# gergely-flamich/compression-without-quantization

Measured on AMD Instinct MI355X. Metric: latent blocks encoded/s at KL=16 bits, higher is better.
Workload: dtype f32

## Files before the change

### compression_without_quantization_amd/build.py

```python
import os
import subprocess
import sys

HERE = os.path.dirname(os.path.abspath(__file__))
CSRC = os.path.join(HERE, "csrc")
OUT = os.path.join(HERE, "libcwq.so")
SOURCES = ["cwq_kernels.hip", "cwq_importance.hip", "cwq_pln.hip", "cwq_partition.hip",
           "cwq_varbits.hip", "cwq_capi.hip", "cwq_ac.cpp"]
HEADERS = ["cwq_math.h", "cwq_screen.h", "cwq_dispatch.h", "cwq_kernels.h", "cwq_device.h",
           "cwq_debug.h"]

FLAGS = ["--offload-arch=gfx950", "-O3", "-std=c++17", "-ffp-contract=off", "-fno-fast-math",
         "-fPIC", "-shared", "-Wall", "-Wno-unused-function"]
LIBS = ["-L/opt/rocm/lib", "-lhsa-runtime64"]


def _stale():
    if not os.path.exists(OUT):
        return True
    t = os.path.getmtime(OUT)
    deps = [os.path.join(CSRC, f) for f in SOURCES + HEADERS]
    deps.append(os.path.join(HERE, "..", "include", "cwq.h"))
    deps.append(os.path.abspath(__file__))
    return any(os.path.getmtime(p) > t for p in deps if os.path.exists(p))


def build(force=False, verbose=True):
    if not force and not _stale():
        return OUT
    cmd = ["hipcc"] + FLAGS + ["-o", OUT] + [os.path.join(CSRC, s) for s in SOURCES] + LIBS
    if verbose:
        print(" ".join(cmd), flush=True)
    subprocess.check_call(cmd)
    return OUT


if __name__ == "__main__":
    build(force="--force" in sys.argv)
```

### compression_without_quantization_amd/csrc/cwq_kernels.hip

```cpp
#include <hip/hip_runtime.h>

#include <type_traits>
#include <stdint.h>

#include "cwq_device.h"
#include "cwq_kernels.h"

namespace cwq {

__global__ void __launch_bounds__(256) k_prep_dims(
    const float* __restrict__ t_scale, const float* __restrict__ p_loc,
    const float* __restrict__ p_scale, int64_t n, float nst, float sdiv, float rho,
    float* __restrict__ loc_s, float* __restrict__ scale_s, float* __restrict__ lognorm,
    float* __restrict__ out_sample, unsigned long long* __restrict__ keys, int64_t nb) {
  for (int64_t g = blockIdx.x * (int64_t)blockDim.x + threadIdx.x; g < nb;
       g += (int64_t)gridDim.x * blockDim.x)
    keys[g] = 0ull;
  for (int64_t i = blockIdx.x * (int64_t)blockDim.x + threadIdx.x; i < n;
       i += (int64_t)gridDim.x * blockDim.x) {
    float ls, ss;
    shard_consts(p_loc[i], p_scale[i], nst, sdiv, rho, ls, ss);
    loc_s[i] = ls;
    scale_s[i] = ss;
    lognorm[i] = lognorm_of(t_scale[i]);
    out_sample[i] = 0.0f;
  }
}

template <int DC, bool STEP0>
__device__ __forceinline__ float eval_row(const PhiloxStream& st, uint64_t kbase, int64_t d_rt,
                                          int align_rt, const float* __restrict__ loc_s,
                                          const float* __restrict__ scale_s,
                                          const float* __restrict__ mu,
                                          const float* __restrict__ sg,
                                          const float* __restrict__ lognorm,
                                          const float* __restrict__ best,
                                          const double* logtab) {
  return eval_row_f<DC>(st, kbase, d_rt, align_rt, logtab, [&](int64_t e, float zz) -> float {
    float s = scale_s[e] * zz;
    s = loc_s[e] + s;
    const float tv = STEP0 ? s : best[e] + s;
    return log_prob(tv, mu[e], sg[e], lognorm[e]);
  });
}

template <int DC, bool STEP0>
__global__ void __launch_bounds__(256) k_encode_eval(
    const float* __restrict__ t_loc, const float* __restrict__ t_scale,
    const float* __restrict__ loc_s, const float* __restrict__ scale_s,
    const float* __restrict__ lognorm, const float* __restrict__ best,
    const int64_t* __restrict__ block_off, int64_t ud, int64_t ntiles, int64_t tiles_per_block,
    int64_t cand_per_tile, int64_t n_cand, SeedSpec sd, int32_t step,
    unsigned long long* __restrict__ keys) {
  __shared__ double logtab[32];
  __shared__ unsigned long long wkey[4];
  fill_logtab(logtab);
  const uint32_t wv = wave_id();
  const uint32_t lane = threadIdx.x & 63u;

  for (int64_t tile = blockIdx.x; tile < ntiles; tile += gridDim.x) {
    const int64_t g = tile / tiles_per_block;
    const int64_t tt = tile - g * tiles_per_block;
    const BlockSpan sp = block_span(block_off, ud, g);
    const int64_t n0 = tt * cand_per_tile;
    const int64_t n1 = (n0 + cand_per_tile < n_cand) ? n0 + cand_per_tile : n_cand;
    const PhiloxStream st =
        generate_key(step_seed(sd.of(g), step), 42);
    const int align = (int)(((uint64_t)(n0 + wv) * (uint64_t)sp.d) & 3u);

    uint64_t bestk = 0;
    for (int64_t n = n0 + 4 * (int64_t)lane + wv; n < n1; n += 256) {
      const float v = eval_row<DC, STEP0>(st, (uint64_t)n * (uint64_t)sp.d, sp.d, align,
                                          loc_s + sp.off, scale_s + sp.off, t_loc + sp.off,
                                          t_scale + sp.off, lognorm + sp.off,
                                          STEP0 ? nullptr : best + sp.off, logtab);
      const uint64_t k = argmax_key(v, (uint32_t)n);
      bestk = k > bestk ? k : bestk;
    }
    bestk = wave_max_u64(bestk);
    if (lane == 0) wkey[wv] = bestk;
    __syncthreads();
    if (threadIdx.x == 0) {
      uint64_t m = wkey[0];
      for (int i = 1; i < 4; ++i) m = wkey[i] > m ? wkey[i] : m;
      if (m) atomicMax(&keys[g], (unsigned long long)m);
    }
    __syncthreads();
  }
}

constexpr float kPruneC1 = 0x1p-14f;
#ifndef CWQ_PRUNE_MIN_WAVES
#define CWQ_PRUNE_MIN_WAVES 6
#endif
#ifndef CWQ_XCD_BALANCE
#define CWQ_XCD_BALANCE 1
#endif
#ifndef CWQ_TAU_SHARE_MASK
#define CWQ_TAU_SHARE_MASK 7u
#endif
#ifndef CWQ_CSR_TAU_SHARE_MASK
#define CWQ_CSR_TAU_SHARE_MASK 15u
#endif
#ifndef CWQ_SURVIVOR_CAP
#define CWQ_SURVIVOR_CAP 1024
#endif

template <bool STEP0>
__device__ __forceinline__ float cand_diff(float z, float ls, float ss, float mu, float bb) {
  const float s = shard_sample(ls, ss, z);
  const float tv = STEP0 ? s : bb + s;
  return tv - mu;
}
__device__ __forceinline__ float lp_from_z(float z, float cc) {
  const float u = -0.5f * (z * z);
  return u - cc;
}


struct VisitRec {
  float4 sa, sb;
  int grp;
  int bk;
  int pad[2];
};
static_assert(sizeof(VisitRec) == 48, "VisitRec: 48 bytes");

template <int D, bool STEP0>
__device__ __forceinline__ float score_rows_wave(
    const PhiloxStream& st, const uint32_t* rows, uint32_t cnt, const float* __restrict__ loc_s,
    const float* __restrict__ scale_s, const float* __restrict__ mu,
    const float* __restrict__ sg, const float* __restrict__ lognorm,
    const float* __restrict__ best, const double* logtab, float* buf, uint32_t lane) {
  constexpr uint32_t G = D / 4;
  const uint32_t r = lane / G, u = lane - r * G;
  if (r < cnt) {
    const F4 z = normal4_dev(st, (uint64_t)rows[r] * G + u, logtab);
#pragma unroll
    for (int t = 0; t < 4; ++t) {
      const uint32_t j = 4u * u + (uint32_t)t;
      const float zz = t == 0 ? z.a : (t == 1 ? z.b : (t == 2 ? z.c : z.d));
      float v = scale_s[j] * zz;
      v = loc_s[j] + v;
      const float tv = STEP0 ? v : best[j] + v;
      buf[r * D + j] = log_prob(tv, mu[j], sg[j], lognorm[j]);
    }
  }
  __builtin_amdgcn_fence(__ATOMIC_SEQ_CST, "wavefront");
  __builtin_amdgcn_wave_barrier();
  float acc = 0.0f;
  const uint32_t fr = lane >> 3;
  if (fr < cnt)
    for (uint32_t e = lane & 7u; e < (uint32_t)D; e += 8u) acc = acc + buf[fr * D + e];
  __builtin_amdgcn_fence(__ATOMIC_SEQ_CST, "wavefront");
  __builtin_amdgcn_wave_barrier();
  float p[8];
#pragma unroll
  for (int l = 0; l < 8; ++l) p[l] = __shfl(acc, (int)((lane & ~7u) + (uint32_t)l), 64);
  return eigen_fold8(p, 0.0f);
}

#ifdef CWQ_TILE_TIMES
constexpr int kTileTimes = 1 << 18;
__device__ unsigned long long g_tile_t0[kTileTimes], g_tile_t1[kTileTimes];
__device__ unsigned int g_tile_wg[kTileTimes];
#endif
#ifdef CWQ_PRUNE_STATS
__device__ unsigned long long g_prune_stats[72];
constexpr int kDbgBlocks = 1 << 20;
__device__ unsigned long long g_dbg_best[kDbgBlocks];
__device__ int g_seed_tau;
#endif

template <int D, bool STEP0, bool INTER>
__global__ void __launch_bounds__(256, CWQ_PRUNE_MIN_WAVES) k_encode_prune(
    const float* __restrict__ t_loc, const float* __restrict__ t_scale,
    const float* __restrict__ loc_s, const float* __restrict__ scale_s,
    const float* __restrict__ lognorm, const float* __restrict__ best, int64_t ntiles,
    int64_t tiles_per_block, int64_t cand_per_tile, int64_t n_cand, SeedSpec sd, int32_t step,
    int allow_screen, unsigned long long* __restrict__ keys, int64_t tail_from, int tail_div,
    uint32_t* __restrict__ tq) {
  static_assert(D % 8 == 0 && D >= 8 && D <= 64, "pruned path: D % 8 == 0, D <= 64");
  constexpr int G = D / 4;
  constexpr int NF = STEP0 ? 6 : 7;
  constexpr int RW = (64 / G) < 8 ? (64 / G) : 8;
  __shared__ double logtab[32];
  __shared__ float4 cst[G * NF];
  __shared__ VisitRec vrec[G];
  __shared__ int2 meta[G];
  __shared__ float rowbuf[4][RW * D];
  __shared__ float dscore[D];
  __shared__ float dA[D];
  __shared__ float dC[D];
  __shared__ float gscore[G];
  __shared__ int gpos[G];
  __shared__ float lowc;
  __shared__ float scr_a, scr_pq;
  __shared__ float tau_cell;
  __shared__ uint32_t sq_cnt;
  __shared__ uint32_t sq_n[CWQ_SURVIVOR_CAP];
  __shared__ float sq_ub[CWQ_SURVIVOR_CAP];
  __shared__ unsigned long long wkey[4];
  __shared__ uint32_t s_next;
#ifdef CWQ_PRUNE_STATS
  __shared__ uint32_t s_ps[72];
  for (int i = threadIdx.x; i < 72; i += blockDim.x) s_ps[i] = 0u;
#endif
  fill_logtab(logtab);
  const uint32_t wv = wave_id();
  const uint32_t lane = threadIdx.x & 63u;

  constexpr bool inter = INTER;
  const int64_t nbt = INTER ? ntiles / tiles_per_block : 0;
  auto next_tile = [&](int64_t cur) -> int64_t {
    if (tq == nullptr) return cur + gridDim.x;
    __syncthreads();
    if (threadIdx.x == 0) s_next = gridDim.x + atomicAdd(tq, 1u);
    __syncthreads();
    return (int64_t)s_next;
  };
  for (int64_t tile = blockIdx.x; tile < ntiles; tile = next_tile(tile)) {
    uint32_t tid = threadIdx.x;
    asm volatile("" : "+v"(tid));
#ifdef CWQ_TILE_TIMES
    if (tid == 0 && tile < kTileTimes) {
      g_tile_t0[tile] = __builtin_amdgcn_s_memrealtime();
      const uint32_t xcc = (uint32_t)__builtin_amdgcn_s_getreg((20) | (0 << 6) | ((4 - 1) << 11));
      g_tile_wg[tile] = (xcc << 24) | (blockIdx.x & 0xffffffu);
    }
#endif
    int64_t tord = tile;
    const int64_t treg = inter ? nbt * tail_from : 0;
    if (inter && CWQ_XCD_BALANCE && tq == nullptr && tile < treg && (treg & 7) == 0 &&
        (gridDim.x & 7u) == 0)
      tord = (tile & 7) * (treg >> 3) + (tile >> 3);
    const int64_t g = inter ? tord % nbt : tile / tiles_per_block;
    const int64_t tt = inter ? tord / nbt : tile - g * tiles_per_block;
    const int64_t off = g * D;
    int64_t n0, csz;
    if (tt < tail_from) {
      n0 = tt * cand_per_tile;
      csz = cand_per_tile;
    } else {
      csz = cand_per_tile / tail_div;
      n0 = tail_from * cand_per_tile + (tt - tail_from) * csz;
    }
    const int64_t n1 = (n0 + csz < n_cand) ? n0 + csz : n_cand;
    if (n0 >= n1) continue;
    const PhiloxStream st =
        generate_key(step_seed(sd.of(g), step), 42);

    if (tid < D) {
      const int j = tid;
      const float ls = loc_s[off + j], ss = scale_s[off + j], mu = t_loc[off + j];
      const float rs = 1.0f / t_scale[off + j];
      const float m = (STEP0 ? ls : best[off + j] + ls) - mu;
      float e = 0.5f * (ss * ss + m * m) * (rs * rs);
      dscore[j] = (e == e) ? e : -1.0f;
    }
    __syncthreads();
    if (tid < G) {
      const int q = tid;
      gscore[q] = ((dscore[4 * q] + dscore[4 * q + 1]) + dscore[4 * q + 2]) + dscore[4 * q + 3];
    }
    __syncthreads();
    if (tid < G) {
      const int q = tid;
      const float sq = gscore[q];
      int r = 0;
      for (int q2 = 0; q2 < G; ++q2) {
        const float s2 = gscore[q2];
        r += (s2 > sq || (s2 == sq && q2 < q)) ? 1 : 0;
      }
      gpos[q] = r;
      meta[r].x = q;
      vrec[r].grp = q;
    }
    __syncthreads();
    int den_ok = 1, scr_ok = 1;
    if (tid < D) {
      const int j = tid, k = gpos[j >> 2], w = j & 3;
      float fj[7];
      const float sgj = t_scale[off + j];
      fj[0] = loc_s[off + j];
      fj[1] = scale_s[off + j];
      fj[2] = t_loc[off + j];
      fj[3] = sgj;
      fj[4] = lognorm[off + j];
      fj[5] = 1.0f / sgj;
      fj[6] = STEP0 ? 0.0f : best[off + j];
      float* c = reinterpret_cast<float*>(cst);
#pragma unroll
      for (int f = 0; f < NF; ++f) c[(k * NF + f) * 4 + w] = fj[f];
      den_ok = markstein_ok_den(sgj) ? 1 : 0;
      const ScreenDim o = screen_dim<STEP0>(fj[0], fj[1], fj[2], sgj, fj[4], fj[6]);
      float* sc = reinterpret_cast<float*>(&vrec[k]);
      sc[w] = o.sa;
      sc[4 + w] = o.sb;
      dA[j] = o.A;
      dC[j] = o.C;
      scr_ok = o.ok ? 1 : 0;
    }
    const bool fastdiv = __syncthreads_and(den_ok) != 0;
    const bool scr_all = __syncthreads_and(scr_ok) != 0;
    const bool screen = allow_screen && scr_all;
    if (tid <= G + 1) {
      const int kb = tid;
      const float* c = reinterpret_cast<const float*>(cst);
      double rf = 0.0, kk = 0.0, asum = 0.0, msum = 0.0, kall = 0.0, cvis = 0.0, a2 = 0.0,
             amax = 0.0;
#pragma unroll 1
      for (int p = 0; p < D; ++p) {
        const double mj = -(double)c[((p >> 2) * NF + 4) * 4 + (p & 3)];
        const double aj = __builtin_fabs(mj);
        asum += aj;
        msum += mj;
        kall += aj + mj;
        if (p >= 4 * kb) {
          rf += mj + 0x1p-17 * aj;
        } else {
          kk += aj + mj;
          if (screen) cvis += (double)dC[(meta[p >> 2].x << 2) + (p & 3)];
        }
        if (screen && kb == G + 1) {
          const double av = (double)dA[p];
          a2 += av * av;
          amax = av > amax ? av : amax;
        }
      }
      const double marg = 0x1p-20 * (__builtin_fabs(rf) + asum) + 0x1p-126;
      const double sl = 0x1p-14 * (__builtin_fabs(msum) + asum + kall) + 0x1p-126;
      if (kb <= G) {
        const float bk = screen ? round_up_f32(msum + cvis * (1.0 + 0x1p-20) + sl)
                                : round_up_f32(rf + 0x1p-14 * kk + marg);
        if (kb >= 1) {
          meta[kb - 1].y = (int)f2u(bk);
          vrec[kb - 1].bk = (int)f2u(bk);
        }
        if (kb == G) lowc = round_up_f32(0x1p-14 * kk + marg);
      } else if (screen) {
        scr_a = screen_as(msum, sl, a2);
        scr_pq = screen_pq(amax, D);
      }
      if (kb == 0) {
        float t0 = -__builtin_inff();
        if (inter) {
          const unsigned long long kv =
              __hip_atomic_load(&keys[g], __ATOMIC_RELAXED, __HIP_MEMORY_SCOPE_AGENT);
          if ((uint32_t)(kv >> 32) > kArgmaxClampOrd) t0 = unord_f32((uint32_t)(kv >> 32));
        }
#ifdef CWQ_PRUNE_STATS
        if (g_seed_tau && g < kDbgBlocks && (g_dbg_best[g] >> 32) > kArgmaxClampOrd)
          t0 = unord_f32((uint32_t)(g_dbg_best[g] >> 32));
#endif
        tau_cell = t0;
        sq_cnt = 0u;
      }
    }
    __syncthreads();
    const float lc = lowc;
#ifdef CWQ_PRUNE_STATS
    const float tau_seed = tau_cell;
#endif
    const float sA = scr_a, sPq = scr_pq;

    const int64_t per_wave = (n1 - n0 + 3) / 4;
    const int64_t w0 = n0 + (int64_t)wv * per_wave;
    const int64_t w1 = (w0 + per_wave < n1) ? w0 + per_wave : n1;
    const uint32_t w0g =
        (uint32_t)__builtin_amdgcn_readfirstlane((int)((uint32_t)w0 * (uint32_t)G));
    const uint32_t ng_end = (uint32_t)__builtin_amdgcn_readfirstlane(
        (int)(w1 > w0 ? (uint32_t)(w1 - w0) * (uint32_t)G : 0u));
#ifndef CWQ_TAU_FROM_KEYS
#define CWQ_TAU_FROM_KEYS 1
#endif
    float tau = (INTER && CWQ_TAU_FROM_KEYS) ? tau_cell : -__builtin_inff();
#ifdef CWQ_PRUNE_STATS
    tau = tau_seed;
#endif
    uint64_t bestk = 0;

    const PhiloxLo lok = philox_lo_key(st);
    auto pass = [&](auto screen_tag) {
      constexpr bool SCREEN = decltype(screen_tag)::value;
      constexpr uint32_t KS = SCREEN ? (uint32_t)sizeof(VisitRec) : 1u;
      uint32_t ng = lane * (uint32_t)G;
      uint32_t wnext_g = 64u * (uint32_t)G;
      uint32_t kp = 0;
      float s = 0.0f;
      uint32_t iter = 0;
      bool active = ng < ng_end;
      uint64_t m_act = __builtin_amdgcn_ballot_w64(active);
      while (m_act != 0ull) {
        int2 mt;
        float4 sa, sb;
        if constexpr (SCREEN) {
          const char* rp = reinterpret_cast<const char*>(vrec) + kp;
          sa = *reinterpret_cast<const float4*>(rp);
          sb = *reinterpret_cast<const float4*>(rp + 16);
          mt = *reinterpret_cast<const int2*>(rp + 32);
        } else {
          mt = meta[kp];
        }
        const uint32_t grp = (ng + (uint32_t)mt.x) + w0g;
        uint32_t pk0 = st.k0, pk1 = st.k1;
        asm volatile("" : "+s"(pk0), "+s"(pk1));
        const U4 x = philox10_lo(grp, lok, pk0, pk1);
        float z0, z1, z2, z3;
        float upper;
        if constexpr (SCREEN) {
          box_muller_screen(x.x, x.y, z0, z1);
          box_muller_screen(x.z, x.w, z2, z3);
          const float a0 = __builtin_fmaf(sa.x, z0, sb.x);
          const float a1 = __builtin_fmaf(sa.y, z1, sb.y);
          const float a2 = __builtin_fmaf(sa.z, z2, sb.z);
          const float a3 = __builtin_fmaf(sa.w, z3, sb.w);
          s = __builtin_fmaf(-a0, a0, s);
          s = __builtin_fmaf(-a1, a1, s);
          s = __builtin_fmaf(-a2, a2, s);
          s = __builtin_fmaf(-a3, a3, s);
          upper = screen_row_upper(s, kScreenC1, u2f((uint32_t)mt.y));
        } else {
          box_muller_dev(x.x, x.y, logtab, z0, z1);
          box_muller_dev(x.z, x.w, logtab, z2, z3);
          const float4* cq = cst + kp * NF;
          const float4 ls = cq[0], ss = cq[1], mu = cq[2], sg = cq[3], cc = cq[4], ry = cq[5];
          const float4 bb = STEP0 ? float4{0.f, 0.f, 0.f, 0.f} : cq[6];
          const float d0 = cand_diff<STEP0>(z0, ls.x, ss.x, mu.x, bb.x);
          const float d1 = cand_diff<STEP0>(z1, ls.y, ss.y, mu.y, bb.y);
          const float d2 = cand_diff<STEP0>(z2, ls.z, ss.z, mu.z, bb.z);
          const float d3 = cand_diff<STEP0>(z3, ls.w, ss.w, mu.w, bb.w);
          float y0 = div_rn_markstein(d0, sg.x, ry.x);
          float y1 = div_rn_markstein(d1, sg.y, ry.y);
          float y2 = div_rn_markstein(d2, sg.z, ry.z);
          float y3 = div_rn_markstein(d3, sg.w, ry.w);
          const bool ok = fastdiv & markstein_ok4(d0, d1, d2, d3);
          if (__builtin_expect(__ballot(!ok) != 0ull, 0)) {
            if (!ok) {
              y0 = d0 / sg.x;
              y1 = d1 / sg.y;
              y2 = d2 / sg.z;
              y3 = d3 / sg.w;
            }
          }
          s = s + lp_from_z(y0, cc.x);
          s = s + lp_from_z(y1, cc.y);
          s = s + lp_from_z(y2, cc.z);
          s = s + lp_from_z(y3, cc.w);
          upper = (s + __builtin_fabsf(s) * kPruneC1) + u2f((uint32_t)mt.y);
        }
        kp += KS;
        const bool complete = (kp == KS * (uint32_t)G);
        const bool below = upper < tau;
        const bool reach = SCREEN ? !below : (upper >= tau);
#ifdef CWQ_PRUNE_STATS
        const bool prune = !complete && below;
        const uint32_t k = kp / KS;
#endif
        const bool done = complete || below || !active;
        const uint64_t m_cpl = __builtin_amdgcn_ballot_w64(complete);
        const uint64_t m_below = __builtin_amdgcn_fcmpf(upper, tau, 4 );
        uint64_t m = m_cpl | m_below | (__builtin_amdgcn_read_exec() & ~m_act);
        uint64_t m_keep =
            m_cpl & m_act &
            (SCREEN ? ~m_below : (uint64_t)__builtin_amdgcn_fcmpf(upper, tau, 3 ));
        asm volatile("" : "+s"(m), "+s"(m_keep));
        if (__builtin_expect(m_keep != 0ull, 0)) {
          const bool keep = complete && active && reach;
          float lower;
          if constexpr (SCREEN)
            lower = screen_row_lower(s, kScreenC2, sA, sPq);
          else
            lower = (s - __builtin_fabsf(s) * kPruneC1) - lc;
          tau = tau_raise_wave(tau, keep, lower);
          if (__builtin_expect(keep && upper >= tau, 0)) {
            uint32_t ngc = ng;
            asm volatile("" : "+v"(ngc));
            const uint32_t n = (w0g + ngc) / (uint32_t)G;
#ifdef CWQ_PRUNE_STATS
            atomicAdd(&s_ps[66], 1u);
#endif
            const uint32_t slot = atomicAdd(&sq_cnt, 1u);
            if (slot < CWQ_SURVIVOR_CAP) {
              sq_n[slot] = (uint32_t)n;
              sq_ub[slot] = upper;
            } else {
#ifdef CWQ_PRUNE_STATS
              atomicAdd(&g_prune_stats[69], 1ull);
#endif
              const float v = eval_row<D, STEP0>(st, (uint64_t)n * D, D, 0, loc_s + off,
                                                 scale_s + off, t_loc + off, t_scale + off,
                                                 lognorm + off, STEP0 ? nullptr : best + off, logtab);
              const uint64_t kv = argmax_key(v, (uint32_t)n);
              bestk = kv > bestk ? kv : bestk;
            }
          }
        }
#ifdef CWQ_PRUNE_STATS
        if (active && (complete || prune)) atomicAdd(&s_ps[k], 1u);
        if (active && complete) atomicAdd(&s_ps[65], 1u);
#endif
        const uint32_t rank = __builtin_amdgcn_mbcnt_hi((uint32_t)(m >> 32),
                                                        __builtin_amdgcn_mbcnt_lo((uint32_t)m, 0u));
        if (done) {
          ng = wnext_g + rank * (uint32_t)G;
          kp = 0;
          s = 0.0f;
        }
        wnext_g += (uint32_t)__builtin_popcountll(m) * (uint32_t)G;
        if (((++iter) & CWQ_TAU_SHARE_MASK) == 0u) tau = tau_share_wave(&tau_cell, tau);
        active = ng < ng_end;
        m_act = __builtin_amdgcn_ballot_w64(active);
      }
    };
#ifdef CWQ_PRUNE_STATS
    if (screen && tid == 0) atomicAdd(&g_prune_stats[67], 1ull);
#endif
    if (screen)
      pass(std::true_type{});
    else
      pass(std::false_type{});

    tau_share_wave(&tau_cell, tau);
    __syncthreads();
    const float tau_final = tau_cell;
    const uint32_t nsurv = sq_cnt < CWQ_SURVIVOR_CAP ? sq_cnt : CWQ_SURVIVOR_CAP;
    const uint32_t nsurv_u = (uint32_t)__builtin_amdgcn_readfirstlane((int)nsurv);
    const uint32_t sl = tid & 63u;
    for (uint32_t c0 = wv * 64u; c0 < nsurv_u; c0 += 256u) {
      const uint32_t i = c0 + sl;
      const bool q = i < nsurv_u && sq_ub[i] >= tau_final;
      const uint32_t nn = i < nsurv_u ? sq_n[i] : 0u;
      const uint64_t qm = __builtin_amdgcn_ballot_w64(q);
      if (qm == 0ull) continue;
#ifdef CWQ_PRUNE_STATS
      if (q) atomicAdd(&g_prune_stats[68], 1ull);
#endif
      const uint32_t qr = __builtin_amdgcn_mbcnt_hi((uint32_t)(qm >> 32),
                                                    __builtin_amdgcn_mbcnt_lo((uint32_t)qm, 0u));
      __builtin_amdgcn_fence(__ATOMIC_SEQ_CST, "wavefront");
      __builtin_amdgcn_wave_barrier();
      if (q) sq_n[c0 + qr] = nn;
      __builtin_amdgcn_fence(__ATOMIC_SEQ_CST, "wavefront");
      __builtin_amdgcn_wave_barrier();
      const uint32_t qn = (uint32_t)__builtin_popcountll(qm);
      for (uint32_t b = 0; b < qn; b += (uint32_t)RW) {
        const uint32_t cnt = qn - b < (uint32_t)RW ? qn - b : (uint32_t)RW;
        const float v = score_rows_wave<D, STEP0>(
            st, sq_n + c0 + b, cnt, loc_s + off, scale_s + off, t_loc + off, t_scale + off,
            lognorm + off, STEP0 ? nullptr : best + off, logtab, rowbuf[wv], sl);
        if ((sl & 7u) == 0u && (sl >> 3) < cnt) {
          const uint64_t kv = argmax_key(v, sq_n[c0 + b + (sl >> 3)]);
          bestk = kv > bestk ? kv : bestk;
        }
      }
    }

    bestk = wave_max_u64(bestk);
    if (lane == 0) wkey[wv] = bestk;
    __syncthreads();
    if (tid == 0) {
      uint64_t mk = wkey[0];
      for (int i = 1; i < 4; ++i) mk = wkey[i] > mk ? wkey[i] : mk;
      if (mk) atomicMax(&keys[g], (unsigned long long)mk);
#ifdef CWQ_PRUNE_STATS
      if (!g_seed_tau && g < kDbgBlocks) g_dbg_best[g] = mk;
#endif
#ifdef CWQ_TILE_TIMES
      if (tile < kTileTimes) g_tile_t1[tile] = __builtin_amdgcn_s_memrealtime();
#endif
    }
#ifdef CWQ_PRUNE_STATS
    if (tid < 72) {
      if (s_ps[tid]) atomicAdd(&g_prune_stats[tid], (unsigned long long)s_ps[tid]);
      s_ps[tid] = 0u;
    }
#endif
    __syncthreads();
  }
}

__device__ __forceinline__ double block_sum_d(double v, double* red) {
  red[threadIdx.x] = v;
  __syncthreads();
  for (int w = 128; w > 0; w >>= 1) {
    if ((int)threadIdx.x < w) red[threadIdx.x] += red[threadIdx.x + w];
    __syncthreads();
  }
  const double r = red[0];
  __syncthreads();
  return r;
}

__host__ __device__ __forceinline__ int64_t csr_cls_stride(int64_t d) { return (d + 6) / 4 + 1; }
constexpr int64_t kCsrSortUnits = 2048;

template <bool STEP0>
__global__ void __launch_bounds__(256) k_csr_prep(
    const float* __restrict__ t_loc, const float* __restrict__ t_scale,
    const float* __restrict__ loc_s, const float* __restrict__ scale_s,
    const float* __restrict__ lognorm, const float* __restrict__ best,
    const int64_t* __restrict__ block_off, int64_t ud, int64_t nb, float2* __restrict__ sab,
    float* __restrict__ cdim, float* __restrict__ bpre, uint32_t* __restrict__ ordu,
    float4* __restrict__ grp, uint32_t* __restrict__ gtau, float4* __restrict__ abp,
    int64_t lds_dims, int64_t coop_min_d) {
  __shared__ double red[5][4];
  __shared__ double wscan[4];
  __shared__ double ucs[256];
  __shared__ unsigned long long skey[kCsrSortUnits];
  const int tid = threadIdx.x;
  const int lane = tid & 63, wv = tid >> 6;
  const bool lead = blockIdx.y == 0;
  for (int64_t g = blockIdx.x; g < nb; g += gridDim.x) {
    const BlockSpan sp = block_span(block_off, ud, g);
    const int64_t off = sp.off, d = sp.d;
    ScreenSums u;
    float2* sabg = sab + off + 8 * g + 4;
    float* cg = cdim + off;
    if (lead && tid < 8) {
      if (tid < 4) sabg[tid - 4] = float2{0.f, 0.f};
      sabg[d + tid] = float2{0.f, 0.f};
    }
    for (int64_t j = tid; j < d; j += 256) {
      const ScreenDim o =
          screen_dim<STEP0>(loc_s[off + j], scale_s[off + j], t_loc[off + j], t_scale[off + j],
                            lognorm[off + j], STEP0 ? 0.0f : best[off + j]);
      sabg[j] = float2{o.sa, o.sb};
      cg[j] = o.C;
      u.add(o);
    }
    u.sm = wave_sum_f64(u.sm);
    u.sa = wave_sum_f64(u.sa);
    u.sk = wave_sum_f64(u.sk);
    u.s2 = wave_sum_f64(u.s2);
    u.mx = wave_max_f64(u.mx);
    if (lane == 0) {
      red[0][wv] = u.sm;
      red[1][wv] = u.sa;
      red[2][wv] = u.sk;
      red[3][wv] = u.s2;
      red[4][wv] = u.mx;
    }
    __threadfence_block();
    const bool all_ok = __syncthreads_and(u.ok) != 0;
    ScreenSums S;
    S.sm = ((red[0][0] + red[0][1]) + red[0][2]) + red[0][3];
    S.sa = ((red[1][0] + red[1][1]) + red[1][2]) + red[1][3];
    S.sk = ((red[2][0] + red[2][1]) + red[2][2]) + red[2][3];
    S.s2 = ((red[3][0] + red[3][1]) + red[3][2]) + red[3][3];
    S.mx = red[4][0];
    for (int w = 1; w < 4; ++w) S.mx = red[4][w] > S.mx ? red[4][w] : S.mx;
    const bool coop_blk = d >= coop_min_d;
    const ScreenBlock bc =
        screen_block_consts(S, d, coop_blk ? 16.0 + (double)d / 64.0 : (double)d);
    const double SM = S.sm, sl = bc.sl;
    const int64_t reg = off + 12 * g, cs = csr_cls_stride(d);
    const bool recs = abp != nullptr && d > lds_dims;
    auto sab_at = [&](int64_t j) {
      const unsigned long long v = __hip_atomic_load(
          reinterpret_cast<unsigned long long*>(sabg + j), __ATOMIC_RELAXED,
          __HIP_MEMORY_SCOPE_AGENT);
      return float2{u2f((uint32_t)v), u2f((uint32_t)(v >> 32))};
    };
    for (int c = (int)blockIdx.y; c < 4; c += (int)gridDim.y) {
      auto unit = [&](int64_t u, double& csum, double& gain) {
        csum = 0.0;
        gain = 0.0;
        for (int t = 0; t < 4; ++t) {
          const int64_t j = 4 * u - c + t;
          if (j >= 0 && j < d) {
            const float2 ab = sab_at(j);
            const float xc = u2f(__hip_atomic_load(reinterpret_cast<uint32_t*>(cg + j),
                                                   __ATOMIC_RELAXED, __HIP_MEMORY_SCOPE_AGENT));
            csum += (double)xc;
            gain += (double)ab.x * (double)ab.x * (0.5 / 0.6931471805599453) +
                    (double)ab.y * (double)ab.y - (double)xc;
          }
        }
      };
      auto key_of = [&](int64_t u) {
        double cu, gu;
        unit(u, cu, gu);
        const float gf = (float)(gu > 0.0 ? gu : 0.0);
        return ((unsigned long long)ord_f32(gf) << 32) | (0xffffffffull - (uint64_t)u);
      };
      const int64_t U = (d + c + 3) / 4;
      const bool sorted = all_ok && U <= kCsrSortUnits;
      const bool small = U <= 256;
      if (sorted && small) {
        unsigned long long key = 0ull;
        if (tid < U) {
          double cu, gu;
          unit(tid, cu, gu);
          ucs[tid] = cu;
          const float gf = (float)(gu > 0.0 ? gu : 0.0);
          key = ((unsigned long long)ord_f32(gf) << 32) | (0xffffffffull - (uint64_t)tid);
          skey[tid] = key;
        }
        __syncthreads();
        int r = 0;
        if (tid < U)
          for (int i = 0; i < (int)U; ++i) r += skey[i] > key ? 1 : 0;
        __syncthreads();
        if (tid < U) skey[r] = key;
        __syncthreads();
      } else if (sorted) {
        int64_t P = 1;
        while (P < U) P <<= 1;
        for (int64_t u = tid; u < P; u += 256) skey[u] = u < U ? key_of(u) : 0ull;
        __syncthreads();
        for (int64_t k = 2; k <= P; k <<= 1) {
          for (int64_t jj = k >> 1; jj > 0; jj >>= 1) {
            for (int64_t i = tid; i < P; i += 256) {
              const int64_t l = i ^ jj;
              if (l > i) {
                const unsigned long long x = skey[i], y = skey[l];
                const bool desc = (i & k) == 0;
                if (desc ? (x < y) : (x > y)) {
                  skey[i] = y;
                  skey[l] = x;
                }
              }
            }
            __syncthreads();
          }
        }
      }
      double carry = 0.0;
      for (int64_t base = 0; base <= U; base += 256) {
        const int64_t k = base + tid;
        int64_t u = k;
        if (sorted && k < U) u = (int64_t)(0xffffffffull - (skey[k] & 0xffffffffull));
        double cu = 0.0, gu;
        if (all_ok && k < U) {
          if (sorted && small)
            cu = ucs[u];
          else
            unit(u, cu, gu);
        }
        if (recs && k <= U) {
          float e[8];
          for (int t = 0; t < 4; ++t) {
            const int64_t j = 4 * u - c + t;
            float2 ab = float2{0.f, 0.f};
            if (k < U && j >= 0 && j < d) ab = sab_at(j);
            e[2 * t] = ab.x;
            e[2 * t + 1] = ab.y;
          }
          float4* rr = abp + 2 * (csr_rec_base(off) + c * cs + k);
          rr[0] = float4{e[0], e[1], e[2], e[3]};
          rr[1] = float4{e[4], e[5], e[6], e[7]};
        }
        double v = cu;
#pragma unroll
        for (int o = 1; o < 64; o <<= 1) {
          const double t = __shfl_up(v, (unsigned)o, 64);
          if (lane >= o) v += t;
        }
        if (lane == 63) wscan[wv] = v;
        __syncthreads();
        double pre = 0.0;
        for (int w = 0; w < wv; ++w) pre += wscan[w];
        const double total = ((wscan[0] + wscan[1]) + wscan[2]) + wscan[3];
        const double excl = carry + (pre + v) - cu;
        if (k <= U) {
          bpre[reg + c * cs + k] = round_up_f32(SM + excl * (1.0 + 0x1p-20) + sl);
          ordu[reg + c * cs + k] = (uint32_t)(k < U ? u : U);
        }
        carry += total;
        __syncthreads();
      }
    }
    if (lead && tid == 0) {
      grp[g] = (all_ok && bc.finite && d > 0) ? float4{bc.c1, bc.c2, bc.as, bc.pq}
                                              : float4{0.f, 0.f, 0.f, 0.f};
      gtau[g * CWQ_CSR_GTAU_STRIDE] = ord_f32(-__builtin_inff());
    }
    __syncthreads();
  }
}

constexpr int kRowChunk = 248;

template <bool STEP0>
__device__ __forceinline__ float exact_row_wave(
    const PhiloxStream& st, uint64_t kbase, int64_t d, const float* __restrict__ loc_s,
    const float* __restrict__ scale_s, const float* __restrict__ mu,
    const float* __restrict__ sg, const float* __restrict__ lognorm,
    const float* __restrict__ best, const double* logtab, float* buf, uint32_t lane) {
  const int64_t vec = d & ~(int64_t)7;
  float acc = 0.0f;
  for (int64_t j0 = 0; j0 < d; j0 += kRowChunk) {
    const int64_t cnt = (d - j0) < kRowChunk ? d - j0 : kRowChunk;
    const uint64_t k0 = kbase + (uint64_t)j0;
    const uint64_t blk = (k0 >> 2) + lane;
    const int64_t ef = (int64_t)(blk << 2) - (int64_t)k0;
    if (ef < cnt) {
      const F4 z = normal4_dev(st, blk, logtab);
#pragma unroll
      for (int t = 0; t < 4; ++t) {
        const int64_t e = ef + t;
        if (e >= 0 && e < cnt) {
          const int64_t j = j0 + e;
          const float zz = t == 0 ? z.a : (t == 1 ? z.b : (t == 2 ? z.c : z.d));
          float v = scale_s[j] * zz;
          v = loc_s[j] + v;
          const float tv = STEP0 ? v : best[j] + v;
          buf[e] = log_prob(tv, mu[j], sg[j], lognorm[j]);
        }
      }
    }
    __builtin_amdgcn_fence(__ATOMIC_SEQ_CST, "wavefront");
    __builtin_amdgcn_wave_barrier();
    if (lane < 8) {
      for (int64_t e = lane; e < cnt && j0 + e < vec; e += 8) acc = acc + buf[e];
// ... 2484 lines not shown
```

Before: 3.573 million.

## Use static per-lane row striding with dynamic refill pool and linked visit records

```diff
diff --git a/compression_without_quantization_amd/build.py b/compression_without_quantization_amd/build.py
--- a/compression_without_quantization_amd/build.py
+++ b/compression_without_quantization_amd/build.py
@@ -8,7 +8,7 @@
 SOURCES = ["cwq_kernels.hip", "cwq_importance.hip", "cwq_pln.hip", "cwq_partition.hip",
            "cwq_varbits.hip", "cwq_capi.hip", "cwq_ac.cpp"]
 HEADERS = ["cwq_math.h", "cwq_screen.h", "cwq_dispatch.h", "cwq_kernels.h", "cwq_device.h",
-           "cwq_debug.h"]
+           "cwq_debug.h", "cwq_refill.h"]
 
 FLAGS = ["--offload-arch=gfx950", "-O3", "-std=c++17", "-ffp-contract=off", "-fno-fast-math",
          "-fPIC", "-shared", "-Wall", "-Wno-unused-function"]
diff --git a/compression_without_quantization_amd/csrc/cwq_kernels.hip b/compression_without_quantization_amd/csrc/cwq_kernels.hip
--- a/compression_without_quantization_amd/csrc/cwq_kernels.hip
+++ b/compression_without_quantization_amd/csrc/cwq_kernels.hip
@@ -5,6 +5,7 @@
 
 #include "cwq_device.h"
 #include "cwq_kernels.h"
+#include "cwq_refill.h"
 
 namespace cwq {
 
@@ -105,6 +106,9 @@
 #ifndef CWQ_SURVIVOR_CAP
 #define CWQ_SURVIVOR_CAP 1024
 #endif
+#ifndef CWQ_LINKED_VISIT
+#define CWQ_LINKED_VISIT 1
+#endif
 
 template <bool STEP0>
 __device__ __forceinline__ float cand_diff(float z, float ls, float ss, float mu, float bb) {
@@ -122,7 +126,8 @@
   float4 sa, sb;
   int grp;
   int bk;
-  int pad[2];
+  int next;
+  int pad;
 };
 static_assert(sizeof(VisitRec) == 48, "VisitRec: 48 bytes");
 
@@ -275,6 +280,7 @@
       gpos[q] = r;
       meta[r].x = q;
       vrec[r].grp = q;
+      vrec[r].next = r + 1 < G ? (r + 1) * (int)sizeof(VisitRec) : 0;
     }
     __syncthreads();
     int den_ok = 1, scr_ok = 1;
@@ -369,8 +375,13 @@
     const int64_t w1 = (w0 + per_wave < n1) ? w0 + per_wave : n1;
     const uint32_t w0g =
         (uint32_t)__builtin_amdgcn_readfirstlane((int)((uint32_t)w0 * (uint32_t)G));
-    const uint32_t ng_end = (uint32_t)__builtin_amdgcn_readfirstlane(
-        (int)(w1 > w0 ? (uint32_t)(w1 - w0) * (uint32_t)G : 0u));
+    const uint32_t wrows = w1 > w0 ? (uint32_t)(w1 - w0) : 0u;
+    const uint32_t ng_end =
+        (uint32_t)__builtin_amdgcn_readfirstlane((int)(wrows * (uint32_t)G));
+    const uint32_t ng_stat = (uint32_t)__builtin_amdgcn_readfirstlane(
+        (int)(cwq::refill_static_rows(wrows) * (uint32_t)G));
+    const uint32_t ng_pool0 = (uint32_t)__builtin_amdgcn_readfirstlane(
+        (int)(cwq::refill_pool_start(cwq::refill_static_rows(wrows)) * (uint32_t)G));
 #ifndef CWQ_TAU_FROM_KEYS
 #define CWQ_TAU_FROM_KEYS 1
 #endif
@@ -384,8 +395,9 @@
     auto pass = [&](auto screen_tag) {
       constexpr bool SCREEN = decltype(screen_tag)::value;
       constexpr uint32_t KS = SCREEN ? (uint32_t)sizeof(VisitRec) : 1u;
+      constexpr bool LINKED = SCREEN && CWQ_LINKED_VISIT;
       uint32_t ng = lane * (uint32_t)G;
-      uint32_t wnext_g = 64u * (uint32_t)G;
+      uint32_t wnext_g = ng_pool0;
       uint32_t kp = 0;
       float s = 0.0f;
       uint32_t iter = 0;
@@ -394,11 +406,14 @@
       while (m_act != 0ull) {
         int2 mt;
         float4 sa, sb;
+        uint32_t kp_next = 0;
         if constexpr (SCREEN) {
           const char* rp = reinterpret_cast<const char*>(vrec) + kp;
           sa = *reinterpret_cast<const float4*>(rp);
           sb = *reinterpret_cast<const float4*>(rp + 16);
-          mt = *reinterpret_cast<const int2*>(rp + 32);
+          const int4 lk = *reinterpret_cast<const int4*>(rp + 32);
+          mt = int2{lk.x, lk.y};
+          kp_next = (uint32_t)lk.z;
         } else {
           mt = meta[kp];
         }
@@ -449,13 +464,16 @@
           s = s + lp_from_z(y3, cc.w);
           upper = (s + __builtin_fabsf(s) * kPruneC1) + u2f((uint32_t)mt.y);
         }
-        kp += KS;
-        const bool complete = (kp == KS * (uint32_t)G);
+        if constexpr (LINKED)
+          kp = kp_next;
+        else
+          kp += KS;
+        const bool complete = LINKED ? (kp == 0u) : (kp == KS * (uint32_t)G);
         const bool below = upper < tau;
         const bool reach = SCREEN ? !below : (upper >= tau);
 #ifdef CWQ_PRUNE_STATS
         const bool prune = !complete && below;
-        const uint32_t k = kp / KS;
+        const uint32_t k = (LINKED && complete) ? (uint32_t)G : kp / KS;
 #endif
         const bool done = complete || below || !active;
         const uint64_t m_cpl = __builtin_amdgcn_ballot_w64(complete);
@@ -500,17 +518,29 @@
         if (active && (complete || prune)) atomicAdd(&s_ps[k], 1u);
         if (active && complete) atomicAdd(&s_ps[65], 1u);
 #endif
-        const uint32_t rank = __builtin_amdgcn_mbcnt_hi((uint32_t)(m >> 32),
-                                                        __builtin_amdgcn_mbcnt_lo((uint32_t)m, 0u));
         if (done) {
-          ng = wnext_g + rank * (uint32_t)G;
+          asm volatile("" : "+v"(ng));
+          ng += 64u * (uint32_t)G;
           kp = 0;
           s = 0.0f;
         }
-        wnext_g += (uint32_t)__builtin_popcountll(m) * (uint32_t)G;
         if (((++iter) & CWQ_TAU_SHARE_MASK) == 0u) tau = tau_share_wave(&tau_cell, tau);
-        active = ng < ng_end;
-        m_act = __builtin_amdgcn_ballot_w64(active);
+        const uint64_t m_pool = m & __builtin_amdgcn_uicmp(ng, ng_stat, 35 );
+        if (m_pool != 0ull) {
+#ifdef CWQ_PRUNE_STATS
+          if (lane == 0) atomicAdd(&s_ps[70], 1u);
+#endif
+          const uint32_t rank = __builtin_amdgcn_mbcnt_hi(
+              (uint32_t)(m_pool >> 32), __builtin_amdgcn_mbcnt_lo((uint32_t)m_pool, 0u));
+          if (done && ng >= ng_stat) ng = wnext_g + rank * (uint32_t)G;
+          wnext_g += (uint32_t)__builtin_popcountll(m_pool) * (uint32_t)G;
+          wnext_g = wnext_g < ng_end ? wnext_g : ng_end;
+          active = ng < ng_end;
+          m_act = __builtin_amdgcn_ballot_w64(active);
+        }
+#ifdef CWQ_PRUNE_STATS
+        if (lane == 0) atomicAdd(&s_ps[71], 1u);
+#endif
       }
     };
 #ifdef CWQ_PRUNE_STATS
diff --git a/compression_without_quantization_amd/csrc/cwq_refill.h b/compression_without_quantization_amd/csrc/cwq_refill.h
--- /dev/null
+++ b/compression_without_quantization_amd/csrc/cwq_refill.h
@@ -0,0 +1,23 @@
+#pragma once
+#include <stdint.h>
+
+#if defined(__HIPCC__)
+#define CWQ_REFILL_HD __host__ __device__ __forceinline__
+#else
+#define CWQ_REFILL_HD inline
+#endif
+
+namespace cwq {
+
+constexpr uint32_t kRefillLanes = 64;
+constexpr uint32_t kRefillMinRows = 128;
+
+CWQ_REFILL_HD uint32_t refill_static_rows(uint32_t R) {
+  if (R < kRefillMinRows) return 0u;
+  const uint32_t s = (uint32_t)(((uint64_t)R * 7u) >> 3);
+  return s & ~(kRefillLanes - 1u);
+}
+
+CWQ_REFILL_HD uint32_t refill_pool_start(uint32_t S) { return S < kRefillLanes ? kRefillLanes : S; }
+
+}
```

New measurement: 3.665 million (median of 6 runs). +2.6%, better.
